# ZJU-FAST-Lab/Implicit-SDF-Planner

Hardware: AMD Instinct MI355X
Metric: SDF cost+grad point-evals/sec (higher is better)
Workload: dtype f64; 1 GPU; V3 ESDF-tile sweep: 1 trajectory x 40 pieces x 65 samples/piece, 256^3 fp32 ESDF @ 0.2 m, kernel_size 21, box robot (1.6,0.3,0.3) central-diff grad, occ_thresh = 0, cull off = BASELINE configs[1]; pieces=40, samples_per_piece=65, grid=256, kernel_size=21, collective=none

## Files before the change

### implicit-sdf-planner_amd/csrc/isdf_host.hip

```cpp
#include "isdf_ctx.hpp"
#include "minco_dev.hpp"
#include "lbfgs_host.hpp"
#include <array>
#include <atomic>
#include <map>
#include <dlfcn.h>
#include <chrono>
#include <cmath>
#include <cstdio>
#include <cstring>
#include <functional>
#include <cstdlib>
#include <string>
#include <vector>
#include <new>
#include "fwn_host.hpp"

using namespace isdf;

namespace {
thread_local std::string g_create_error;
}

int isdf_fail(isdf_ctx *c, int code, const char *msg) {
// ... 731 lines not shown
static int rebuild_bit_grids(isdf_ctx *c, const isdf_config &cfg, SweepParams &P, hipStream_t st) {
    const int zw = (c->grid.Z + 31) / 32, xw = (c->grid.X + 31) / 32, yw = (c->grid.Y + 31) / 32;
    const size_t nwz = (size_t)c->grid.X * c->grid.Y * zw, nwx = (size_t)c->grid.Y * c->grid.Z * xw, nwy = (size_t)c->grid.X * c->grid.Z * yw;
    { const int rc = c->d_bits.reserve(c, nwz + nwx + nwy); if (rc) return rc; }
    c->grid.ZW = zw; c->grid.XW = xw; c->grid.YW = yw;
    c->grid.bits = c->d_bits; c->grid.bits_x = c->d_bits + nwz; c->grid.bits_y = c->d_bits + nwz + nwx;
    launch_build_bits(c->grid, cfg.variant == ISDF_V3_ESDF_TILE ? 1 : 0, cfg.occ_thresh, c->d_bits, st);
    launch_build_bits_xy(c->grid, cfg.variant == ISDF_V3_ESDF_TILE ? 1 : 0, cfg.occ_thresh, c->d_bits + nwz, c->d_bits + nwz + nwx, st);
    c->bits_dirty = false;
    P.grid = c->grid;
    return ISDF_OK;
}

static int plan_order(isdf_ctx *c, const isdf_config &cfg, SweepParams &P, bool fused, long long pb, long long pe, long long total_pieces, hipStream_t st) {
    const int N = P.N;
    P.plan_cls_in = nullptr; P.plan_cls_out = nullptr; P.plan_map_out = nullptr; P.plan_zone = 0; P.plan_group = 1;
    P.plan_lr_in = P.plan_hist_in = nullptr; P.plan_lr_out = P.plan_hist_out = nullptr;
    const int K1 = cfg.integral_intervs + 1;
    const long long n_loc = pe - pb, ns_local = n_loc * K1;
    const int nb = (int)((ns_local + 3) / 4);
    P.n_sweep_blocks = nb;
    if (c->n_cus == 0) { hipDeviceProp_t pr; c->n_cus = (hipGetDeviceProperties(&pr, c->device) == hipSuccess && pr.multiProcessorCount > 0) ? pr.multiProcessorCount : 256; }
    const bool no_plan = c->env_no_lpt;
    bool plan = cfg.enable_pos && !no_plan && !P.sample_map && K1 <= 128 && nb > c->n_cus && ns_local < (1LL << 28) && c->shape.kind != ISDF_SHAPE_MESH;
    long long group = n_loc;
    int zone = 0;
    if (plan) {
        if (fused) {
            plan = P.xf.world <= 1 && pb == 0 && pe == total_pieces && ns_local <= PLAN_GROUP_MAX_SAMPLES;
            zone = c->n_cus;
        } else if (nb <= sweep_resident_blocks(P, c->n_cus) && ns_local <= PLAN_GROUP_MAX_SAMPLES) {
// ... 10 lines not shown
        c->plan_ns_cap = c->plan_np_cap = 0; c->plan_k = 0; c->plan_cur = 0;
        const size_t nsc = std::max(ns_cap, (size_t)4096), npc = std::max(np_cap, (size_t)256);
        HIPCHK(c, c->d_plan_cls.alloc(2 * nsc));
        HIPCHK(c, c->d_plan_map.alloc(2 * nsc));
        HIPCHK(c, c->d_plan_lr.alloc(2 * nsc));
        HIPCHK(c, c->d_plan_hist.alloc(2 * npc * PLAN_CLASSES));
        c->plan_ns_cap = nsc; c->plan_np_cap = npc;
    }
    const long long geo = ((long long)n_loc << 32) | ((long long)K1 << 20) | ((long long)(fused ? 1 : 0) << 19) | (long long)(group & 0x7FFFF);
    if (c->plan_ns != ns_local || c->plan_nb != nb || c->plan_geo != geo) { c->plan_k = 0; c->plan_ns = ns_local; c->plan_nb = nb; c->plan_geo = geo; }
    constexpr int PLAN_CYCLE = 8;
    const int k = c->plan_k, ph = k % PLAN_CYCLE;
    const size_t nsc = c->plan_ns_cap;
    P.plan_zone = zone;
    P.plan_group = (int)group;
    if (ph == 0) P.plan_cls_out = c->d_plan_cls;
    if (ph == 1) { P.plan_cls_in = c->d_plan_cls; P.plan_lr_out = c->d_plan_lr; P.plan_hist_out = c->d_plan_hist; }
    if (ph == 2) { P.plan_lr_in = c->d_plan_lr; P.plan_hist_in = c->d_plan_hist; P.plan_map_out = c->d_plan_map + (size_t)(1 - c->plan_cur) * nsc; }
    if (ph == 3) c->plan_cur = 1 - c->plan_cur;
    if (k >= 3) P.sample_map = c->d_plan_map + (size_t)c->plan_cur * nsc;
    if (c->plan_k < (1 << 30)) c->plan_k++;
    return ISDF_OK;
}

static int mesh_queue(isdf_ctx *c, const isdf_config &cfg, SweepParams &P, size_t ns_loc) {
    const double k3 = (double)cfg.kernel_size * cfg.kernel_size * cfg.kernel_size;
    double vox = k3;
    if (c->shape.prune_rows) {
        double v = 1.0;
        for (int a = 0; a < 3; a++) v *= ((double)c->shape.bbox_hi[a] - (double)c->shape.bbox_lo[a] + 2.2 * cfg.safety_hor) / P.grid.res + 3.0;
// ... 61 lines not shown
    P.bd_half = cfg.kernel_size * P.grid.res / 2;
    P.safety_hor = cfg.safety_hor; P.weight_p = cfg.weight_p; P.weight_v = cfg.weight_v; P.weight_omg = cfg.weight_omg;
    P.weight_theta = cfg.weight_theta;
    P.vel_sqr_max = cfg.vmax * cfg.vmax; P.omg_sqr_max = cfg.omgmax * cfg.omgmax; P.theta_max = cfg.thetamax;
    P.mu = cfg.smoothing_eps; P.inv_mu = 1.0 / cfg.smoothing_eps; P.inv_K = 1.0 / cfg.integral_intervs;
    P.occ_thresh = (float)cfg.occ_thresh;
    P.cull_threshold = 0.0;
    if (cfg.variant == ISDF_V3_ESDF_TILE && cfg.enable_cull && c->shape.bound_radius > 0)
        P.cull_threshold = c->shape.bound_radius + cfg.safety_hor + std::sqrt(3.0) * P.grid.res + (cfg.occ_thresh > 0 ? cfg.occ_thresh : 0.0);
    P.T = d_T; P.coeffs = d_coeffs; P.acc = c->d_acc; P.sample_info = c->d_sample_info; P.piece_cost = c->d_piece_cost;
    P.out = d_out; P.stats = c->d_stats;
    P.dbg = nullptr;
    P.sample_map = (c->d_sample_map && c->sample_map_n == 4 * ((ns_loc + 3) / 4)) ? c->d_sample_map.get() : nullptr;
    P.dbg_flags = 0;
    if (const char *e = getenv("ISDF_DEBUG_FLAGS")) P.dbg_flags = atoi(e);
    rc = debug_timing_buffer(c, n_samples * 8 + (size_t)total_pieces * 4 + 4, st, &P.dbg);
    if (rc) return rc;
    if (cfg.enable_pos && c->bits_dirty) { rc = rebuild_bit_grids(c, cfg, P, st); if (rc) return rc; }
    c->last_P = P; c->have_last_P = true;
    ProfEvent *ev;
    rc = prof_begin(c, st, &ev);
    if (rc) return rc;
    if (ev && !cfg.enable_pos) { ev = nullptr; c->prof_used--; }
    const bool ev2 = ev && c->prof_secondary;
    const bool fused = c->fuse_small && !ev2 && sweep_can_fuse(P);
    {
        int xerr = ISDF_OK;
        if (isdf_xchg_fill(c, &P.xf, (size_t)total_pieces, &xerr)) {
            if (xerr != ISDF_OK) return xerr;
        }
    }
// ... 1078 lines not shown
    (void)hipSetDevice(c->device);
    (void)hipDeviceSynchronize();
    c->d_sample_map.release(); c->sample_map_n = 0;
    if (!map || n <= 0) return ISDF_OK;
    if (c->d_sample_map.alloc((size_t)n) != hipSuccess) return ISDF_ERR_HIP;
    (void)hipMemcpy(c->d_sample_map, map, (size_t)n * sizeof(int), hipMemcpyHostToDevice);
    c->sample_map_n = (size_t)n;
    return ISDF_OK;
}

extern "C" int isdf_debug_plan_map(isdf_ctx *c, int *out, long long cap) {
    if (!c || c->plan_k < 4 || !c->d_plan_map) return 0;
    (void)hipSetDevice(c->device);
    (void)hipDeviceSynchronize();
    const long long n = 4LL * c->plan_nb < cap ? 4LL * c->plan_nb : cap;
    if (out && n > 0) (void)hipMemcpy(out, c->d_plan_map + (size_t)c->plan_cur * c->plan_ns_cap, (size_t)n * sizeof(int), hipMemcpyDeviceToHost);
    return c->plan_k;
}

extern "C" long long isdf_debug_sample_info(isdf_ctx *c, int *out, long long cap) {
    if (!c || !c->d_sample_info || !c->have_last_P) return 0;
    (void)hipSetDevice(c->device);
    (void)hipDeviceSynchronize();
    const long long n = (long long)(c->last_P.piece_end - c->last_P.piece_begin) * (c->last_P.K + 1);
    const long long m = 2 * n < cap ? 2 * n : cap;
    if (out && m > 0) (void)hipMemcpy(out, c->d_sample_info, (size_t)m * sizeof(int), hipMemcpyDeviceToHost);
    return n;
}

extern "C" const char *isdf_debug_peek_hip_error(void) { return hipGetErrorString(hipPeekAtLastError()); }
```

### implicit-sdf-planner_amd/csrc/isdf_internal.hpp

```cpp
#pragma once
#include <hip/hip_runtime.h>
#include <hip/hip_ext.h>
#include <cstdint>
#include "dev_shapes.hpp"

namespace isdf {

struct DevGrid {
    int X, Y, Z;
    double res;
    double bmin[3], bmax[3];
    const float *esdf;
    const uint8_t *occ;
    const unsigned *bits;
    int ZW;
    const unsigned *bits_x;
    const unsigned *bits_y;
    int XW, YW;
};
constexpr int PLAN_CLASSES = 8;
constexpr int PLAN_GROUP_MAX_SAMPLES = 65535;
constexpr int ACC_STRIDE = 8;
constexpr int PARTIAL_STRIDE = 20;
constexpr int SWEPT_MAX_COARSE = 1536;
// ... 36 lines not shown
    unsigned long long *stats;
    const double *host_T, *host_coeffs;
    double *stage;
    unsigned long long *stage_flags;
    unsigned long long seq;
    unsigned long long *host_flag;
    void *poses;
    const int *sample_map;
    unsigned char *plan_cls_out;
    const unsigned char *plan_cls_in;
    unsigned short *plan_lr_out, *plan_hist_out;
    const unsigned short *plan_lr_in, *plan_hist_in;
    int *plan_map_out;
    int plan_zone;
    int plan_group;
    int dbg_flags;
    unsigned long long *dbg;
    unsigned *mq_entries;
    int2 *mq_items;
    double *mq_res;
    int *mq_sample_items;
    int *mq_sample_n;
    unsigned *mq_count;
    unsigned mq_cap;
    int mq_kmax;
};

size_t sweep_pose_bytes();
bool sweep_can_fuse(const SweepParams &P);
int sweep_resident_blocks(const SweepParams &P, int n_cus);
// ... 47 lines not shown
```

### implicit-sdf-planner_amd/csrc/tile_sweep.hip

```cpp
#define ISDF_LEAN_MATH 1
#ifndef ISDF_SWEEP_STATS
#define ISDF_SWEEP_STATS 0
#endif
#include "isdf_internal.hpp"
#include "dev_mesh.hpp"

namespace isdf {

constexpr int SW_LIST_CAP = 1024;
constexpr int MQ_BLOCK = 16;
constexpr int SW_PASS = 8;
constexpr int SW_NEAR_CAP = 512;
constexpr float TS_FILTER_EPS = 2e-3f;

__device__ __forceinline__ void wave_lds_sync() {
    __builtin_amdgcn_fence(__ATOMIC_RELEASE, "wavefront");
    __builtin_amdgcn_wave_barrier();
    __builtin_amdgcn_fence(__ATOMIC_ACQUIRE, "wavefront");
}

__device__ __forceinline__ bool in_map(const DevGrid &G, double x, double y, double z) {
    if (x < G.bmin[0] || y < G.bmin[1] || z < G.bmin[2]) return false;
    if (x > G.bmax[0] || y > G.bmax[1] || z > G.bmax[2]) return false;
    return true;
// ... 229 lines not shown
    const int n3 = nb - Z, p1 = pos - q0, w = p1 / n3;
    return w * nb + Z + (p1 - w * n3);
}
__device__ __forceinline__ uint4 plan_add(uint4 a, uint4 b) {
    return make_uint4(a.x + b.x, a.y + b.y, a.z + b.z, a.w + b.w);
}
__device__ __forceinline__ uint4 plan_wave_sum(uint4 v) {
#pragma unroll
    for (int d = 1; d < 64; d <<= 1) v = plan_add(v, make_uint4(__shfl_xor(v.x, d), __shfl_xor(v.y, d), __shfl_xor(v.z, d), __shfl_xor(v.w, d)));
    return v;
}
__device__ __forceinline__ unsigned plan_count(uint4 v, int q) {
    const unsigned w = (q >> 1) == 0 ? v.x : (q >> 1) == 1 ? v.y : (q >> 1) == 2 ? v.z : v.w;
    return (w >> (16 * (q & 1))) & 0xFFFFu;
}
__device__ void plan_wave(const SweepParams &P, const int t, const int lane) {
    const int K1 = P.K + 1, n_pieces = P.piece_end - P.piece_begin;
    const int ns = n_pieces * K1, nb = P.n_sweep_blocks, Z = P.plan_zone;
    const int G = P.plan_group, gp0 = (t / G) * G, gn = min(G, n_pieces - gp0);
    const int s0 = t * K1 + lane, s1 = s0 + 64;
    const bool h0 = lane < K1, h1 = lane + 64 < K1;
    if (P.plan_cls_in) {
        const int c0 = h0 ? (int)(P.plan_cls_in[s0] & (PLAN_CLASSES - 1)) : -1, c1 = h1 ? (int)(P.plan_cls_in[s1] & (PLAN_CLASSES - 1)) : -1;
        int r0 = 0, r1 = 0, hist = 0;
        const unsigned long long lt = (1ull << lane) - 1ull;
#pragma unroll
        for (int q = 0; q < PLAN_CLASSES; q++) {
            const unsigned long long m0 = __ballot(c0 == q), m1 = __ballot(c1 == q);
            if (c0 == q) r0 = __popcll(m0 & lt);
            if (c1 == q) r1 = __popcll(m0) + __popcll(m1 & lt);
// ... 9 lines not shown
            const uint4 h = reinterpret_cast<const uint4 *>(P.plan_hist_in)[i];
            tot = plan_add(tot, h);
            if (i < t) bef = plan_add(bef, h);
        }
        tot = plan_wave_sum(tot); bef = plan_wave_sum(bef);
        int base = 0;
        if (lane < PLAN_CLASSES) {
            base = (int)plan_count(bef, lane);
#pragma unroll
            for (int q = 1; q < PLAN_CLASSES; q++) if (q > lane) base += (int)plan_count(tot, q);
        }
        const unsigned v0 = h0 ? P.plan_lr_in[s0] : 0u, v1 = h1 ? P.plan_lr_in[s1] : 0u;
        const int b0 = __shfl(base, (int)(v0 & 7u)), b1 = __shfl(base, (int)(v1 & 7u));
        const int p0 = gp0 * K1 + b0 + (int)(v0 >> 3), p1 = gp0 * K1 + b1 + (int)(v1 >> 3);
        if (Z > 0) {
            if (h0) P.plan_map_out[plan_rank(p0, Z, nb)] = s0;
            if (h1) P.plan_map_out[plan_rank(p1, Z, nb)] = s1;
            if (t == 0) for (int pos = ns + lane; pos < 4 * nb; pos += 64) P.plan_map_out[plan_rank(pos, Z, nb)] = -1;
        } else {
            if (h0) P.plan_map_out[(p0 & 3) * nb + (p0 >> 2)] = s0;
            if (h1) P.plan_map_out[(p1 & 3) * nb + (p1 >> 2)] = s1;
            if (t == 0) for (int pos = ns + lane; pos < 4 * nb; pos += 64) P.plan_map_out[(pos & 3) * nb + (pos >> 2)] = -1;
        }
    }
}

constexpr int POSE_THREADS = 64;
constexpr int POSE_REC = (int)(sizeof(SweepPose) / 8);
__global__ __launch_bounds__(POSE_THREADS) void pose_kernel(const SweepParams P) {
    __shared__ double s_rec[POSE_THREADS][POSE_REC + 1];
    const int K1 = P.K + 1;
    const long long s_begin = (long long)P.piece_begin * K1, s_end = (long long)P.piece_end * K1;
// ... 77 lines not shown
    const int v0 = sa_w == 2 ? w0[1] : w0[2], v1 = sa_w == 2 ? w1[1] : w1[2];
    sp.rx0 = (flags_w & 1) ? u0 : 0; sp.ry0 = (flags_w & 1) ? v0 : 0;
    sp.rnx = (flags_w & 1) ? max(0, u1 - u0 + 1) : 0; sp.rny = (flags_w & 1) ? max(0, v1 - v0 + 1) : 0;
    sp.nzt = sa_w == 2 ? nn[2] : (sa_w == 0 ? nn[0] : nn[1]);
    sp.flags = flags_w;
    sp.sa = sa_w;
    scan_consts(P, scan_launch_consts(P, P.shape.kind), sp.pos, sp.R, sp.lo, sa_w, sp.rny, P.shape.kind == ISDF_SHAPE_ROUNDEDCONE && P.shape.f.ident != 0, sp);
    }
    __syncthreads();
    const int n_rec = (int)min((long long)POSE_THREADS, s_end - s_first);
    double *dst = (double *)((SweepPose *)P.poses + (s_first - s_begin));
    for (int i = threadIdx.x; i < n_rec * POSE_REC; i += POSE_THREADS) dst[i] = s_rec[i / POSE_REC][i % POSE_REC];
}
size_t sweep_pose_bytes() { return sizeof(SweepPose); }

template <bool EARLY, bool XF> __device__ __forceinline__ void tail_piece(const SweepParams &P, const int t, double (*s_val)[PARTIAL_STRIDE + 1]);

template <int KIND, bool IDENT, bool FUSED>
__global__ __launch_bounds__(64 * SW_SAMPLES, FUSED ? 3 : sweep_waves_per_simd(KIND, IDENT)) void sweep_kernel(const SweepParams P) {
    const int n_blocks = FUSED ? P.n_sweep_blocks : (int)gridDim.x;
    if constexpr (FUSED) {
        __shared__ double s_tail[TL_THREADS][PARTIAL_STRIDE + 1];
        if ((int)blockIdx.x >= n_blocks) {
            if ((P.plan_cls_in || P.plan_lr_in) && !(P.dbg_flags & 2) && (threadIdx.x >> 6) == SW_SAMPLES - 1) plan_wave(P, (int)blockIdx.x - n_blocks, threadIdx.x & 63);
            if (P.xf.world > 1) tail_piece<false, true>(P, (int)blockIdx.x - n_blocks, s_tail);
            else tail_piece<false, false>(P, (int)blockIdx.x - n_blocks, s_tail);
            return;
        }
    }
    if constexpr (FUSED) {
        if (P.host_T && (int)blockIdx.x < (P.n_traj * P.N + STAGE_G - 1) / STAGE_G) stage_in(P, (int)blockIdx.x);
    }
    __shared__ SweepPose s_pose[SW_SAMPLES];
    __shared__ unsigned s_list[SW_SAMPLES][SW_LIST_CAP];
    __shared__ unsigned s_near[SW_SAMPLES][SW_NEAR_CAP];
    __shared__ __attribute__((aligned(16))) int s_plan[SW_SAMPLES][4];
    __shared__ double s_res[SW_SAMPLES][SW_NEAR_CAP / 64][ACC_STRIDE];
    __shared__ int s_resn[SW_SAMPLES][SW_NEAR_CAP / 64][2];
    __shared__ __attribute__((aligned(8))) unsigned s_mframes[KIND == ISDF_SHAPE_MESH ? SW_SAMPLES : 1][KIND == ISDF_SHAPE_MESH ? mesh_frames_words(MESH_Q_LEVELS) : 2];

    const int lane = threadIdx.x & 63;
    const int wave = __builtin_amdgcn_readfirstlane(threadIdx.x >> 6);
    const int K1 = P.K + 1;
    const long long s_begin = (long long)P.piece_begin * K1, s_end = (long long)P.piece_end * K1;
    const DevGrid &G = P.grid;
    const long long rank_w = (long long)blockIdx.x + (long long)wave * n_blocks;
    long long sidx = s_begin + rank_w;
    if (P.sample_map) { const int m = __builtin_amdgcn_readfirstlane(P.sample_map[rank_w]); sidx = m >= 0 ? s_begin + m : s_end; }
    unsigned long long *const dbg = (ISDF_SWEEP_STATS && P.dbg && sidx < s_end) ? P.dbg + (size_t)(sidx - s_begin) * 8 : nullptr;
    if (dbg && lane == 0) { dbg[0] = wall_clock64(); dbg[1] = clock64(); }

    auto sample_of_rank = [&](long long rank) -> long long {
        if (P.sample_map) { const int m = P.sample_map[rank]; return m >= 0 ? s_begin + m : s_end; }
        return s_begin + rank;
    };
    if constexpr (FUSED) {
    long long pose_sidx = s_end;
    if (wave == 0 && lane < SW_SAMPLES) pose_sidx = sample_of_rank((long long)blockIdx.x + (long long)lane * n_blocks);
    if (pose_sidx < s_end) {
        const SampleId id = decode_sample(P, pose_sidx);
        bool staged = true;
        if constexpr (FUSED) if (P.host_T) staged = stage_wait(P, id.b * P.N + id.i);
        if (!staged && P.stats) atomicMax(&P.stats[4], 1ull);
        const PieceIn pin = piece_in(P, id.b, id.i);
        const double *c = pin.c;
        const int ld = pin.ld;
        const double step = pin.T * P.inv_K;
        Basis B;
        poly_basis(id.j * step, B);
        const d3 pos = ct_beta(c, ld, B.b0), vel = ct_beta<1>(c, ld, B.b1), acc = ct_beta<2>(c, ld, B.b2);
        FlatS fs;
        flat_core(P.flat, vel, acc, fs);
        const d4 quat = flat_quat(fs);
        const m3 R = quat_to_rot(quat);
        SweepPose &sp = s_pose[lane];
        sp.pos[0] = pos.x; sp.pos[1] = pos.y; sp.pos[2] = pos.z;
#pragma unroll
        for (int k = 0; k < 9; k++) sp.R[k] = R.a[k];
        sp.quat[0] = quat.w; sp.quat[1] = quat.x; sp.quat[2] = quat.y; sp.quat[3] = quat.z;
        int flags = 0;
        if (P.enable_pos) {
            flags = 1;
// ... 6 lines not shown
            const double hb[3] = {0.5 * ((double)P.shape.bbox_hi[0] - (double)P.shape.bbox_lo[0]) + infl,
                                  0.5 * ((double)P.shape.bbox_hi[1] - (double)P.shape.bbox_lo[1]) + infl,
                                  0.5 * ((double)P.shape.bbox_hi[2] - (double)P.shape.bbox_lo[2]) + infl};
            const double cb[3] = {0.5 * ((double)P.shape.bbox_hi[0] + (double)P.shape.bbox_lo[0]),
                                  0.5 * ((double)P.shape.bbox_hi[1] + (double)P.shape.bbox_lo[1]),
                                  0.5 * ((double)P.shape.bbox_hi[2] + (double)P.shape.bbox_lo[2])};
            const double p[3] = {pos.x, pos.y, pos.z};
#pragma unroll
            for (int a = 0; a < 3; a++) {
                const double ctr = p[a] + R.a[3 * a] * cb[0] + R.a[3 * a + 1] * cb[1] + R.a[3 * a + 2] * cb[2];
                const double ext = fabs(R.a[3 * a]) * hb[0] + fabs(R.a[3 * a + 1]) * hb[1] + fabs(R.a[3 * a + 2]) * hb[2];
                sp.L0[a] = (ctr - ext - G.bmin[a]) * inv_res - 0.5;
                sp.L1[a] = (ctr + ext - G.bmin[a]) * inv_res - 0.5;
            }
        }
    }
    if (wave == 1 && lane < 3 * SW_SAMPLES && P.enable_pos) {
        const int ps = lane / 3, a = lane - 3 * ps;
        const long long sx = sample_of_rank((long long)blockIdx.x + (long long)ps * n_blocks);
        if (sx < s_end) {
            const SampleId id = decode_sample(P, sx);
            if constexpr (FUSED) if (P.host_T) (void)stage_wait(P, id.b * P.N + id.i);
            const PieceIn pin = piece_in(P, id.b, id.i);
            const double step = pin.T * P.inv_K;
            Basis B;
            poly_basis(id.j * step, B);
            const double *ca = pin.c + (size_t)a * pin.ld;
            double pa = 0.0;
#pragma unroll
            for (int k = 0; k < 6; k++) pa += ca[k] * B.b0[k];
            const double bmn = a == 0 ? G.bmin[0] : (a == 1 ? G.bmin[1] : G.bmin[2]), bmx = a == 0 ? G.bmax[0] : (a == 1 ? G.bmax[1] : G.bmax[2]);
            const int dim = a == 0 ? G.X : (a == 1 ? G.Y : G.Z);
            const int lo = axis_index(clampd(pa - P.bd_half, bmn, bmx), bmn, G.res, dim);
            const int hi = axis_index(clampd(pa + P.bd_half, bmn, bmx), bmn, G.res, dim);
            s_pose[ps].lo[a] = lo;
            s_pose[ps].nn[a] = hi - lo + 1;
// ... 118 lines not shown
        for (int a = 0; a < 3; a++) { Ru[a] = w.Ru[a]; Rv[a] = w.Rv[a]; Rw[a] = w.Rw[a]; dzv[a] = w.dzv[a]; dzi[a] = w.dzi[a]; }
        pv_u = w.pvu; pv_v = w.pvv; pv_w = w.pvw; inv_rny = w.inv_rny;
        cone_alpha = w.cone_alpha; cone_ia = w.cone_ia; cone_on = w.cone_on != 0;
    } else {
#pragma unroll
        for (int k = 0; k < 9; k++) Rf[k] = rec->Rf[k];
        pvx = rec->pv[0]; pvy = rec->pv[1]; pvz = rec->pv[2];
#pragma unroll
        for (int a = 0; a < 3; a++) { Ru[a] = rec->Ru[a]; Rv[a] = rec->Rv[a]; Rw[a] = rec->Rw[a]; dzv[a] = rec->dzv[a]; dzi[a] = rec->dzi[a]; }
        pv_u = rec->pvu; pv_v = rec->pvv; pv_w = rec->pvw; inv_rny = rec->inv_rny;
        cone_alpha = rec->cone_alpha; cone_ia = rec->cone_ia; cone_on = rec->cone_on != 0;
#pragma unroll
        for (int a = 0; a < 3; a++) { asm volatile("" : "+v"(dzv[a])); asm volatile("" : "+v"(dzi[a])); }
    }
    const float cone_A = SL.cone_A, cone_B = SL.cone_B;

    auto row_xy = [&](int t) -> unsigned {
        unsigned wx = (unsigned)((float)t * inv_rny);
        int rem = t - (int)wx * rny;
        if (rem < 0) { wx--; rem += rny; } else if (rem >= rny) { wx++; rem -= rny; }
        const unsigned wy = (unsigned)rem;
        return ((wx + (unsigned)rx0) << sh_u) | ((wy + (unsigned)ry0) << sh_v);
    };
    auto row_bits = [&](unsigned pk, int zb) -> unsigned {
        const int z0 = lo_w + (zb << 5);
        const int nz = min(32, nzt - (zb << 5));
        const size_t rowbase = ((size_t)(lo_u + (int)((pk >> sh_u) & 1023u)) * dim_v + (lo_v + (int)((pk >> sh_v) & 1023u))) * n_ww;
        const int w0 = z0 >> 5, sh = z0 & 31;
        const unsigned b0 = bits_a[rowbase + w0];
        const unsigned b1 = bits_a[rowbase + min(w0 + 1, n_ww - 1)];
// ... 478 lines not shown
    const int K1 = P.K + 1;
    const long long n_samples = (long long)(P.piece_end - P.piece_begin) * K1;
    unsigned long long culled = 0, pairs = 0, grads = 0;
    if (P.enable_pos)
        for (long long s = (long long)blockIdx.x * blockDim.x + threadIdx.x; s < n_samples; s += (long long)gridDim.x * blockDim.x) {
            const int a = P.sample_info[2 * s], b = P.sample_info[2 * s + 1];
            pairs += (unsigned)a; grads += (unsigned)(b & 0x7fffffff);
            if (b < 0) culled++;
        }
    if (culled) atomicAdd(&P.stats[1], culled);
    if (pairs) atomicAdd(&P.stats[2], pairs);
    if (grads) atomicAdd(&P.stats[3], grads);
    if (blockIdx.x == 0 && threadIdx.x == 0) atomicAdd(&P.stats[0], (unsigned long long)n_samples);
}

template <bool EARLY, bool XF> __device__ __forceinline__ void tail_piece(const SweepParams &P, const int t, double (*s_val)[PARTIAL_STRIDE + 1]) {
    const int K1 = P.K + 1;
    const int tid = threadIdx.x;
    const int n_own = P.piece_end - P.piece_begin;
    int gp = t;
    if constexpr (XF) gp = t < n_own ? P.piece_begin + t : (t - n_own < P.piece_begin ? t - n_own : t);
    const int b = gp / P.N, i = gp - b * P.N;
    const size_t ostride = (size_t)1 + 19 * (size_t)P.N;
    const int p0 = max(P.piece_begin, b * P.N) - b * P.N, p1 = min(P.piece_end, (b + 1) * P.N) - b * P.N;
    double *const o = P.out + (size_t)b * ostride;
    double *const my_board = XF ? P.xf.board[P.xf.rank] + (size_t)P.xf.parity * P.xf.parity_stride : nullptr;
    bool lost = false;
    const bool mine = i >= p0 && i < p1;
    unsigned long long *const dbg = (ISDF_SWEEP_STATS && P.dbg && mine) ? P.dbg + (size_t)(P.piece_end - P.piece_begin) * K1 * 8 + (size_t)(gp - P.piece_begin) * 4 : nullptr;
    if (!mine) {
        const int q = tid;
        if constexpr (XF) {
            if (q < 19) {
                double v;
                unsigned long long deadline = 0ull;
                lost = !xslot_take(my_board + (size_t)gp * XF_ROW + q, v, P.xf.timeout_ticks, deadline);
                if (q == 18) o[1 + i] = v;
                else { const int d = q / 6, r = q - 6 * d; o[1 + P.N + (size_t)d * 6 * P.N + 6 * i + r] = v; }
            }
        } else {
            if (q == 18) o[1 + i] = 0.0;
            else if (q < 18) { const int d = q / 6, r = q - 6 * d; o[1 + P.N + (size_t)d * 6 * P.N + 6 * i + r] = 0.0; }
            else if (q == 19 && p1 <= p0 && i == 0) o[0] = 0.0;
            return;
// ... 1 lines not shown
    } else {
    if constexpr (!EARLY) {
        if (P.host_T) {
            __shared__ int s_staged;
            if (tid == 0) s_staged = stage_wait(P, gp) ? 1 : 0;
            __syncthreads();
            lost = lost || !s_staged;
        }
    }
    const PieceIn pin = piece_in(P, b, i);
    const double *c = pin.c;
    const int ld = pin.ld;
    const double integral_frac = P.inv_K;
    const double step = pin.T * integral_frac;
    double colsum = 0.0;
    unsigned long long tl_c0 = 0, tl_marks = 0;
    if (dbg && tid == 0) { dbg[0] = wall_clock64(); tl_c0 = clock64(); }
#define TL_MARK(k) do { if (dbg && tid == 0) tl_marks |= (((clock64() - tl_c0) >> 4) & 0xFFFFull) << (16 * (k)); } while (0)
    for (int j0 = 0; j0 < (EARLY ? K1 : min(K1, 1)); j0 += TL_THREADS) {
        const int j = j0 + tid;
        if (tid < TL_THREADS && j < K1) {
            const long long s = (long long)gp * K1 + j;
            double *const ap = P.acc + (size_t)(s - (long long)P.piece_begin * K1) * ACC_STRIDE;
            double ab[EARLY ? ACC_STRIDE : 1];
            if (EARLY && P.enable_pos) {
#pragma unroll
                for (int q = 0; q < ACC_STRIDE; q++) ab[q] = ap[q];
            }
            d3 vel, acc3, jer0;
            {
                Basis B;
                poly_basis(j * step, B);
                vel = ct_beta<1>(c, ld, B.b1); acc3 = ct_beta<2>(c, ld, B.b2); jer0 = ct_beta<3>(c, ld, B.b3);
            }
            TL_MARK(0);
            double pena = 0.0;
            d3 gradVel = mk3(0, 0, 0), gradPos = gradVel, gradOmg = gradVel;
            d4 gradQuat; gradQuat.w = gradQuat.x = gradQuat.y = gradQuat.z = 0.0;
            FlatS fs; FlatS2 ft;
            flat_core(P.flat, vel, acc3, fs);
            flat_core2(P.flat, vel, acc3, jer0, fs, ft);
            if (P.enable_dyn) {
                const d4 quat = flat_quat(fs);
                const d3 omg = flat_omg(fs, ft);
                const double cos_theta = 1.0 - 2.0 * (quat.x * quat.x + quat.y * quat.y);
                const double violaVel = dot3(vel, vel) - P.vel_sqr_max;
                const double violaOmg = dot3(omg, omg) - P.omg_sqr_max;
                const double violaTheta = acos(cos_theta) - P.theta_max;
// ... 35 lines not shown
                }
                if (a[0] > 0.0) {
                    gradPos.x += P.weight_p * a[1]; gradPos.y += P.weight_p * a[2]; gradPos.z += P.weight_p * a[3];
                    gradQuat.w += P.weight_p * a[4]; gradQuat.x += P.weight_p * a[5];
                    gradQuat.y += P.weight_p * a[6]; gradQuat.z += P.weight_p * a[7];
                    pena += P.weight_p * a[0];
                }
            }
            d3 gP, gV, gA, gJ;
            TL_MARK(2);
            flat_backward_from(P.flat, vel, acc3, fs, ft, gradPos, gradVel, gradQuat, gradOmg, gP, gV, gA, gJ);
            TL_MARK(3);
            const double node = (j == 0 || j == P.K) ? 0.5 : 1.0;
            const double alpha = j * integral_frac;
            double *o = s_val[tid];
            double s1 = j * step;
            asm volatile("" : "+v"(s1));
            Basis B;
            poly_basis(s1, B);
            const d3 jer = ct_beta<3>(c, ld, B.b3), sna = ct_beta<4>(c, ld, B.b4);
            const double gPv[3] = {gP.x, gP.y, gP.z}, gVv[3] = {gV.x, gV.y, gV.z}, gAv[3] = {gA.x, gA.y, gA.z}, gJv[3] = {gJ.x, gJ.y, gJ.z};
#pragma unroll
            for (int d = 0; d < 3; d++)
#pragma unroll
                for (int r = 0; r < 6; r++) {
                    double v = B.b0[r] * gPv[d];
                    if (r >= 1) v += B.b1[r] * gVv[d];
                    if (r >= 2) v += B.b2[r] * gAv[d];
                    if (r >= 3) v += B.b3[r] * gJv[d];
                    o[d * 6 + r] = v * node * step;
                }
            o[18] = (dot3(gP, vel) + dot3(gV, acc3) + dot3(gA, jer) + dot3(gJ, sna)) * alpha * node * step + node * integral_frac * pena;
            o[19] = node * step * pena;
        }
        __syncthreads();
        {
            const int n = min(TL_THREADS, K1 - j0);
            const int col = tid % PARTIAL_STRIDE, grp = tid / PARTIAL_STRIDE;
            double part = 0.0;
            if (grp < TL_GROUPS) for (int row = grp; row < n; row += TL_GROUPS) part += s_val[row][col];
            __syncthreads();
            if (grp < TL_GROUPS) s_val[grp][col] = part;
            __syncthreads();
            if (tid < PARTIAL_STRIDE) {
#pragma unroll
                for (int g = 0; g < TL_GROUPS; g++) colsum += s_val[g][tid];
            }
        }
        __syncthreads();
    }
    if (dbg && tid == 0) { dbg[2] = tl_marks; dbg[3] = (clock64() - tl_c0) >> 4; }
#undef TL_MARK
    if (P.host_flag) lost = __syncthreads_or(lost ? 1 : 0) != 0;
    if (tid < PARTIAL_STRIDE) {
        const int q = tid;
        if (q < 19) {
            if (q == 18) o[1 + i] = colsum;
            else { const int d = q / 6, r = q - 6 * d; o[1 + P.N + (size_t)d * 6 * P.N + 6 * i + r] = colsum; }
            if constexpr (XF) {
                for (int r = 0; r < P.xf.world; r++)
                    if (r != P.xf.rank) xslot_publish(P.xf.board[r] + (size_t)P.xf.parity * P.xf.parity_stride + (size_t)gp * XF_ROW + q, colsum);
            }
        } else {
            if (P.host_flag) { if (lost && P.stats) atomicMax(&P.stats[4], 1ull); __builtin_amdgcn_fence(__ATOMIC_RELEASE, ""); }
            if constexpr (XF) {
                for (int r = 0; r < P.xf.world; r++) xslot_publish(P.xf.board[r] + (size_t)P.xf.parity * P.xf.parity_stride + (size_t)gp * XF_ROW + 19, colsum);
            } else slot_publish(&P.piece_cost[gp], colsum);
        }
    }
    }
    if (lost && P.stats) atomicMax(&P.stats[4], 1ull);
    bool collector;
    int k0, k1;
    if constexpr (XF) {
        const int first = b * P.N, last = first + P.N - 1;
        const int t_last = (last >= P.piece_begin && last < P.piece_end) ? last - P.piece_begin : (last < P.piece_begin ? last + n_own : last);
        const int below = P.piece_begin - 1;
        const int t_below = (below >= first && below <= last) ? below + n_own : -1;
        collector = t == max(t_last, t_below);
        k0 = 0; k1 = P.N;
    } else {
        collector = i == p1 - 1;
        k0 = p0; k1 = p1;
    }
// ... 16 lines not shown
                v = __longlong_as_double((long long)bits);
            }
            sum += v;
        }
        sum = wave_sum(sum);
        if (__ballot(gone) != 0ull) { sum = __longlong_as_double(0x7FF8000000000000ll); if (tid == 0 && P.stats) atomicMax(&P.stats[4], 1ull); }
        if (tid == 0) o[0] = sum;
    }
    if constexpr (!XF) {
        if (P.host_flag && collector && tid == 0) {
            __builtin_amdgcn_fence(__ATOMIC_ACQUIRE, "agent");
            const unsigned long long ovf = P.stats ? __hip_atomic_load(&P.stats[4], __ATOMIC_RELAXED, __HIP_MEMORY_SCOPE_AGENT) : 0ull;
            __hip_atomic_store(&P.host_flag[b], P.seq | (ovf ? HOST_FLAG_OVERFLOW : 0ull), __ATOMIC_RELEASE, __HIP_MEMORY_SCOPE_SYSTEM);
        }
    }
    if (dbg && tid == 0) dbg[1] = wall_clock64();
}

constexpr int TL_LAUNCH_THREADS = TL_THREADS + 64;
template <bool XF> __device__ __forceinline__ void tail_plan(const SweepParams &P) {
    if (!(P.plan_cls_in || P.plan_lr_in) || (P.dbg_flags & 2) || (int)(threadIdx.x >> 6) != TL_THREADS / 64) return;
    int gp = (int)blockIdx.x;
    if constexpr (XF) { const int n_own = P.piece_end - P.piece_begin, t = gp; gp = t < n_own ? P.piece_begin + t : (t - n_own < P.piece_begin ? t - n_own : t); }
    if (gp >= P.piece_begin && gp < P.piece_end) plan_wave(P, gp - P.piece_begin, (int)(threadIdx.x & 63));
}
__global__ __launch_bounds__(TL_LAUNCH_THREADS) void tail_kernel(const SweepParams P) {
    __shared__ double s_val[TL_THREADS][PARTIAL_STRIDE + 1];
    tail_plan<false>(P);
    tail_piece<true, false>(P, (int)blockIdx.x, s_val);
}
__global__ __launch_bounds__(TL_LAUNCH_THREADS) void tail_kernel_xf(const SweepParams P) {
    __shared__ double s_val[TL_THREADS][PARTIAL_STRIDE + 1];
    tail_plan<true>(P);
    tail_piece<true, true>(P, (int)blockIdx.x, s_val);
}

static int fused_max_blocks() {
    static const int v = [] { const char *e = getenv("ISDF_FUSE_MAX_BLOCKS"); const int n = e ? atoi(e) : 0; return n > 0 ? n : 3 * 256; }();
    return v;
}

int sweep_resident_blocks(const SweepParams &P, int n_cus) {
    const bool ident = P.shape.d.ident != 0;
    const int kind = P.shape.kind == ISDF_SHAPE_MESH ? ISDF_SHAPE_MESH : P.shape.kind;
    return sweep_waves_per_simd(kind, kind == ISDF_SHAPE_MESH ? false : ident) * n_cus;
}

bool sweep_can_fuse(const SweepParams &P) {
    if (!P.enable_pos || P.shape.kind == ISDF_SHAPE_MESH || P.shape.d.ident == 0) return false;
// ... 105 lines not shown
```

Baseline: 162.4 million point-evals/s.

## Pack plan map entries, park tail basis values in LDS, overlay fused tail reduction

In fused mode, each plan-map entry is now packed as (piece<<7)|sample, so the sweep can get piece and sample indices with shifts and no integer division. The fused tail stores the polynomial basis terms and the jerk/snap vectors in its shared-memory row during the first pass, so the second pass reuses them instead of recomputing the basis. Its reduction writes partial sums into the otherwise unused s_res buffer, which the sweep's large shared arrays now share, and this removes two __syncthreads barriers. It also adds debug timing marks, which are compiled only when stats are enabled.

```diff
diff --git a/implicit-sdf-planner_amd/csrc/isdf_host.hip b/implicit-sdf-planner_amd/csrc/isdf_host.hip
--- a/implicit-sdf-planner_amd/csrc/isdf_host.hip
+++ b/implicit-sdf-planner_amd/csrc/isdf_host.hip
@@ -769,7 +769,7 @@
 
 static int plan_order(isdf_ctx *c, const isdf_config &cfg, SweepParams &P, bool fused, long long pb, long long pe, long long total_pieces, hipStream_t st) {
     const int N = P.N;
-    P.plan_cls_in = nullptr; P.plan_cls_out = nullptr; P.plan_map_out = nullptr; P.plan_zone = 0; P.plan_group = 1;
+    P.plan_cls_in = nullptr; P.plan_cls_out = nullptr; P.plan_map_out = nullptr; P.plan_zone = 0; P.plan_group = 1; P.plan_packed = 0;
     P.plan_lr_in = P.plan_hist_in = nullptr; P.plan_lr_out = P.plan_hist_out = nullptr;
     const int K1 = cfg.integral_intervs + 1;
     const long long n_loc = pe - pb, ns_local = n_loc * K1;
@@ -810,6 +810,7 @@
     const size_t nsc = c->plan_ns_cap;
     P.plan_zone = zone;
     P.plan_group = (int)group;
+    P.plan_packed = (fused && n_loc < (1LL << 23)) ? 1 : 0;
     if (ph == 0) P.plan_cls_out = c->d_plan_cls;
     if (ph == 1) { P.plan_cls_in = c->d_plan_cls; P.plan_lr_out = c->d_plan_lr; P.plan_hist_out = c->d_plan_hist; }
     if (ph == 2) { P.plan_lr_in = c->d_plan_lr; P.plan_hist_in = c->d_plan_hist; P.plan_map_out = c->d_plan_map + (size_t)(1 - c->plan_cur) * nsc; }
@@ -901,7 +902,7 @@
     P.sample_map = (c->d_sample_map && c->sample_map_n == 4 * ((ns_loc + 3) / 4)) ? c->d_sample_map.get() : nullptr;
     P.dbg_flags = 0;
     if (const char *e = getenv("ISDF_DEBUG_FLAGS")) P.dbg_flags = atoi(e);
-    rc = debug_timing_buffer(c, n_samples * 8 + (size_t)total_pieces * 4 + 4, st, &P.dbg);
+    rc = debug_timing_buffer(c, n_samples * 12 + (size_t)total_pieces * 8 + 4, st, &P.dbg);
     if (rc) return rc;
     if (cfg.enable_pos && c->bits_dirty) { rc = rebuild_bit_grids(c, cfg, P, st); if (rc) return rc; }
     c->last_P = P; c->have_last_P = true;
@@ -2010,7 +2011,12 @@
     (void)hipSetDevice(c->device);
     (void)hipDeviceSynchronize();
     const long long n = 4LL * c->plan_nb < cap ? 4LL * c->plan_nb : cap;
-    if (out && n > 0) (void)hipMemcpy(out, c->d_plan_map + (size_t)c->plan_cur * c->plan_ns_cap, (size_t)n * sizeof(int), hipMemcpyDeviceToHost);
+    if (out && n > 0) {
+        (void)hipMemcpy(out, c->d_plan_map + (size_t)c->plan_cur * c->plan_ns_cap, (size_t)n * sizeof(int), hipMemcpyDeviceToHost);
+        const int K1 = (int)((c->plan_geo >> 20) & 0xFFF);
+        if ((c->plan_geo >> 19) & 1)
+            for (long long i = 0; i < n; i++) if (out[i] >= 0) out[i] = (out[i] >> 7) * K1 + (out[i] & 127);
+    }
     return c->plan_k;
 }
 
diff --git a/implicit-sdf-planner_amd/csrc/isdf_internal.hpp b/implicit-sdf-planner_amd/csrc/isdf_internal.hpp
--- a/implicit-sdf-planner_amd/csrc/isdf_internal.hpp
+++ b/implicit-sdf-planner_amd/csrc/isdf_internal.hpp
@@ -74,6 +74,7 @@
     int *plan_map_out;
     int plan_zone;
     int plan_group;
+    int plan_packed;
     int dbg_flags;
     unsigned long long *dbg;
     unsigned *mq_entries;
diff --git a/implicit-sdf-planner_amd/csrc/tile_sweep.hip b/implicit-sdf-planner_amd/csrc/tile_sweep.hip
--- a/implicit-sdf-planner_amd/csrc/tile_sweep.hip
+++ b/implicit-sdf-planner_amd/csrc/tile_sweep.hip
@@ -267,6 +267,7 @@
     const unsigned w = (q >> 1) == 0 ? v.x : (q >> 1) == 1 ? v.y : (q >> 1) == 2 ? v.z : v.w;
     return (w >> (16 * (q & 1))) & 0xFFFFu;
 }
+__device__ __forceinline__ int plan_entry_sample(const SweepParams &P, int m, int K1) { return P.plan_packed ? (m >> 7) * K1 + (m & 127) : m; }
 __device__ void plan_wave(const SweepParams &P, const int t, const int lane) {
     const int K1 = P.K + 1, n_pieces = P.piece_end - P.piece_begin;
     const int ns = n_pieces * K1, nb = P.n_sweep_blocks, Z = P.plan_zone;
@@ -306,8 +307,8 @@
         const int b0 = __shfl(base, (int)(v0 & 7u)), b1 = __shfl(base, (int)(v1 & 7u));
         const int p0 = gp0 * K1 + b0 + (int)(v0 >> 3), p1 = gp0 * K1 + b1 + (int)(v1 >> 3);
         if (Z > 0) {
-            if (h0) P.plan_map_out[plan_rank(p0, Z, nb)] = s0;
-            if (h1) P.plan_map_out[plan_rank(p1, Z, nb)] = s1;
+            if (h0) P.plan_map_out[plan_rank(p0, Z, nb)] = P.plan_packed ? ((t << 7) | lane) : s0;
+            if (h1) P.plan_map_out[plan_rank(p1, Z, nb)] = P.plan_packed ? ((t << 7) | (lane + 64)) : s1;
             if (t == 0) for (int pos = ns + lane; pos < 4 * nb; pos += 64) P.plan_map_out[plan_rank(pos, Z, nb)] = -1;
         } else {
             if (h0) P.plan_map_out[(p0 & 3) * nb + (p0 >> 2)] = s0;
@@ -415,17 +416,23 @@
 }
 size_t sweep_pose_bytes() { return sizeof(SweepPose); }
 
-template <bool EARLY, bool XF> __device__ __forceinline__ void tail_piece(const SweepParams &P, const int t, double (*s_val)[PARTIAL_STRIDE + 1]);
+template <bool EARLY, bool XF> __device__ __forceinline__ void tail_piece(const SweepParams &P, const int t, double (*s_val)[PARTIAL_STRIDE + 1], double *s_part);
+constexpr int TL_PARK = 20;
+static_assert(TL_PARK <= PARTIAL_STRIDE, "a thread parks in its own row");
 
 template <int KIND, bool IDENT, bool FUSED>
 __global__ __launch_bounds__(64 * SW_SAMPLES, FUSED ? 3 : sweep_waves_per_simd(KIND, IDENT)) void sweep_kernel(const SweepParams P) {
     const int n_blocks = FUSED ? P.n_sweep_blocks : (int)gridDim.x;
+    __shared__ unsigned s_list[SW_SAMPLES][SW_LIST_CAP];
+    __shared__ unsigned s_near[SW_SAMPLES][SW_NEAR_CAP];
+    __shared__ double s_res[SW_SAMPLES][SW_NEAR_CAP / 64][ACC_STRIDE];
     if constexpr (FUSED) {
         __shared__ double s_tail[TL_THREADS][PARTIAL_STRIDE + 1];
         if ((int)blockIdx.x >= n_blocks) {
             if ((P.plan_cls_in || P.plan_lr_in) && !(P.dbg_flags & 2) && (threadIdx.x >> 6) == SW_SAMPLES - 1) plan_wave(P, (int)blockIdx.x - n_blocks, threadIdx.x & 63);
-            if (P.xf.world > 1) tail_piece<false, true>(P, (int)blockIdx.x - n_blocks, s_tail);
-            else tail_piece<false, false>(P, (int)blockIdx.x - n_blocks, s_tail);
+            static_assert(sizeof(s_res) >= TL_GROUPS * (PARTIAL_STRIDE + 1) * 8, "overlay of the fused tail");
+            if (P.xf.world > 1) tail_piece<false, true>(P, (int)blockIdx.x - n_blocks, s_tail, &s_res[0][0][0]);
+            else tail_piece<false, false>(P, (int)blockIdx.x - n_blocks, s_tail, &s_res[0][0][0]);
             return;
         }
     }
@@ -433,10 +440,7 @@
         if (P.host_T && (int)blockIdx.x < (P.n_traj * P.N + STAGE_G - 1) / STAGE_G) stage_in(P, (int)blockIdx.x);
     }
     __shared__ SweepPose s_pose[SW_SAMPLES];
-    __shared__ unsigned s_list[SW_SAMPLES][SW_LIST_CAP];
-    __shared__ unsigned s_near[SW_SAMPLES][SW_NEAR_CAP];
     __shared__ __attribute__((aligned(16))) int s_plan[SW_SAMPLES][4];
-    __shared__ double s_res[SW_SAMPLES][SW_NEAR_CAP / 64][ACC_STRIDE];
     __shared__ int s_resn[SW_SAMPLES][SW_NEAR_CAP / 64][2];
     __shared__ __attribute__((aligned(8))) unsigned s_mframes[KIND == ISDF_SHAPE_MESH ? SW_SAMPLES : 1][KIND == ISDF_SHAPE_MESH ? mesh_frames_words(MESH_Q_LEVELS) : 2];
 
@@ -447,19 +451,34 @@
     const DevGrid &G = P.grid;
     const long long rank_w = (long long)blockIdx.x + (long long)wave * n_blocks;
     long long sidx = s_begin + rank_w;
-    if (P.sample_map) { const int m = __builtin_amdgcn_readfirstlane(P.sample_map[rank_w]); sidx = m >= 0 ? s_begin + m : s_end; }
+    if (P.sample_map) { const int m = __builtin_amdgcn_readfirstlane(P.sample_map[rank_w]); sidx = m >= 0 ? s_begin + plan_entry_sample(P, m, K1) : s_end; }
     unsigned long long *const dbg = (ISDF_SWEEP_STATS && P.dbg && sidx < s_end) ? P.dbg + (size_t)(sidx - s_begin) * 8 : nullptr;
     if (dbg && lane == 0) { dbg[0] = wall_clock64(); dbg[1] = clock64(); }
-
-    auto sample_of_rank = [&](long long rank) -> long long {
-        if (P.sample_map) { const int m = P.sample_map[rank]; return m >= 0 ? s_begin + m : s_end; }
-        return s_begin + rank;
+    [[maybe_unused]] const auto dbg_ext = [&](long long s) -> unsigned long long * {
+        return P.dbg + (size_t)(s_end - s_begin) * 8 + (size_t)(P.piece_end - P.piece_begin) * 4 + 4 + (size_t)(s - s_begin) * 4;
+    };
+
+    [[maybe_unused]] auto sample_of_rank = [&](long long rank) -> SampleId {
+        if (P.sample_map && P.plan_packed) {
+            const int m = P.sample_map[rank];
+            SampleId id;
+            const int gp = P.piece_begin + (m >> 7);
+            id.j = m & 127;
+            id.b = P.n_traj == 1 ? 0 : gp / P.N;
+            id.i = gp - id.b * P.N;
+            id.s = m >= 0 ? (long long)gp * K1 + id.j : s_end;
+            return id;
+        }
+        long long s = s_begin + rank;
+        if (P.sample_map) { const int m = P.sample_map[rank]; s = m >= 0 ? s_begin + m : s_end; }
+        return decode_sample(P, s);
     };
     if constexpr (FUSED) {
-    long long pose_sidx = s_end;
-    if (wave == 0 && lane < SW_SAMPLES) pose_sidx = sample_of_rank((long long)blockIdx.x + (long long)lane * n_blocks);
+    SampleId id;
+    id.s = s_end; id.b = id.i = id.j = 0;
+    if (wave == 0 && lane < SW_SAMPLES) id = sample_of_rank((long long)blockIdx.x + (long long)lane * n_blocks);
+    const long long pose_sidx = id.s;
     if (pose_sidx < s_end) {
-        const SampleId id = decode_sample(P, pose_sidx);
         bool staged = true;
         if constexpr (FUSED) if (P.host_T) staged = stage_wait(P, id.b * P.N + id.i);
         if (!staged && P.stats) atomicMax(&P.stats[4], 1ull);
@@ -467,6 +486,14 @@
         const double *c = pin.c;
         const int ld = pin.ld;
         const double step = pin.T * P.inv_K;
+#if ISDF_SWEEP_STATS
+        if (P.dbg) {
+            double all = step;
+            for (int d = 0; d < 3; d++) for (int k = 0; k < 6; k++) all += c[(size_t)d * ld + k];
+            asm volatile("" :: "v"(all));
+            dbg_ext(pose_sidx)[0] = clock64();
+        }
+#endif
         Basis B;
         poly_basis(id.j * step, B);
         const d3 pos = ct_beta(c, ld, B.b0), vel = ct_beta<1>(c, ld, B.b1), acc = ct_beta<2>(c, ld, B.b2);
@@ -503,12 +530,14 @@
                 sp.L1[a] = (ctr + ext - G.bmin[a]) * inv_res - 0.5;
             }
         }
+#if ISDF_SWEEP_STATS
+        if (P.dbg) { asm volatile("s_waitcnt lgkmcnt(0)" ::: "memory"); dbg_ext(pose_sidx)[1] = clock64(); }
+#endif
     }
     if (wave == 1 && lane < 3 * SW_SAMPLES && P.enable_pos) {
         const int ps = lane / 3, a = lane - 3 * ps;
-        const long long sx = sample_of_rank((long long)blockIdx.x + (long long)ps * n_blocks);
-        if (sx < s_end) {
-            const SampleId id = decode_sample(P, sx);
+        const SampleId id = sample_of_rank((long long)blockIdx.x + (long long)ps * n_blocks);
+        if (id.s < s_end) {
             if constexpr (FUSED) if (P.host_T) (void)stage_wait(P, id.b * P.N + id.i);
             const PieceIn pin = piece_in(P, id.b, id.i);
             const double step = pin.T * P.inv_K;
@@ -657,6 +686,9 @@
         for (int a = 0; a < 3; a++) { asm volatile("" : "+v"(dzv[a])); asm volatile("" : "+v"(dzi[a])); }
     }
     const float cone_A = SL.cone_A, cone_B = SL.cone_B;
+#if ISDF_SWEEP_STATS
+    if (dbg && lane == 0 && !primed) { float all = pvx + pvy + pvz + pv_u + pv_v + pv_w + inv_rny + dzi[0] + dzi[1] + dzi[2] + cone_ia; asm volatile("" :: "v"(all)); dbg_ext(sidx)[2] = clock64(); }
+#endif
 
     auto row_xy = [&](int t) -> unsigned {
         unsigned wx = (unsigned)((float)t * inv_rny);
@@ -1165,7 +1197,7 @@
     if (blockIdx.x == 0 && threadIdx.x == 0) atomicAdd(&P.stats[0], (unsigned long long)n_samples);
 }
 
-template <bool EARLY, bool XF> __device__ __forceinline__ void tail_piece(const SweepParams &P, const int t, double (*s_val)[PARTIAL_STRIDE + 1]) {
+template <bool EARLY, bool XF> __device__ __forceinline__ void tail_piece(const SweepParams &P, const int t, double (*s_val)[PARTIAL_STRIDE + 1], double *s_part) {
     const int K1 = P.K + 1;
     const int tid = threadIdx.x;
     const int n_own = P.piece_end - P.piece_begin;
@@ -1179,6 +1211,8 @@
     bool lost = false;
     const bool mine = i >= p0 && i < p1;
     unsigned long long *const dbg = (ISDF_SWEEP_STATS && P.dbg && mine) ? P.dbg + (size_t)(P.piece_end - P.piece_begin) * K1 * 8 + (size_t)(gp - P.piece_begin) * 4 : nullptr;
+    [[maybe_unused]] unsigned long long *const dbg2 = dbg ? P.dbg + (size_t)n_own * K1 * 12 + (size_t)n_own * 4 + 4 + (size_t)(gp - P.piece_begin) * 4 : nullptr;
+    [[maybe_unused]] unsigned long long tl_c0 = 0, tl_marks2 = 0;
     if (!mine) {
         const int q = tid;
         if constexpr (XF) {
@@ -1210,9 +1244,10 @@
     const double integral_frac = P.inv_K;
     const double step = pin.T * integral_frac;
     double colsum = 0.0;
-    unsigned long long tl_c0 = 0, tl_marks = 0;
+    unsigned long long tl_marks = 0;
     if (dbg && tid == 0) { dbg[0] = wall_clock64(); tl_c0 = clock64(); }
 #define TL_MARK(k) do { if (dbg && tid == 0) tl_marks |= (((clock64() - tl_c0) >> 4) & 0xFFFFull) << (16 * (k)); } while (0)
+#define TL_MARK2(k) do { if (ISDF_SWEEP_STATS && dbg && tid == 0) tl_marks2 |= (((clock64() - tl_c0) >> 4) & 0xFFFFull) << (16 * (k)); } while (0)
     for (int j0 = 0; j0 < (EARLY ? K1 : min(K1, 1)); j0 += TL_THREADS) {
         const int j = j0 + tid;
         if (tid < TL_THREADS && j < K1) {
@@ -1228,6 +1263,13 @@
                 Basis B;
                 poly_basis(j * step, B);
                 vel = ct_beta<1>(c, ld, B.b1); acc3 = ct_beta<2>(c, ld, B.b2); jer0 = ct_beta<3>(c, ld, B.b3);
+                if constexpr (!EARLY) {
+                    const d3 sna0 = ct_beta<4>(c, ld, B.b4);
+                    const double pk[TL_PARK] = {B.b0[1], B.b0[2], B.b0[3], B.b0[4], B.b0[5], B.b1[2], B.b1[3], B.b1[4], B.b1[5], B.b2[3], B.b2[4], B.b2[5],
+                                                B.b3[4], B.b3[5], jer0.x, jer0.y, jer0.z, sna0.x, sna0.y, sna0.z};
+#pragma unroll
+                    for (int k = 0; k < TL_PARK; k++) s_val[tid][k] = pk[k];
+                }
             }
             TL_MARK(0);
             double pena = 0.0;
@@ -1293,11 +1335,24 @@
             const double node = (j == 0 || j == P.K) ? 0.5 : 1.0;
             const double alpha = j * integral_frac;
             double *o = s_val[tid];
-            double s1 = j * step;
-            asm volatile("" : "+v"(s1));
             Basis B;
-            poly_basis(s1, B);
-            const d3 jer = ct_beta<3>(c, ld, B.b3), sna = ct_beta<4>(c, ld, B.b4);
+            d3 jer, sna;
+            if constexpr (EARLY) {
+                double s1 = j * step;
+                asm volatile("" : "+v"(s1));
+                poly_basis(s1, B);
+                jer = ct_beta<3>(c, ld, B.b3); sna = ct_beta<4>(c, ld, B.b4);
+            } else {
+                double pk[TL_PARK];
+#pragma unroll
+                for (int k = 0; k < TL_PARK; k++) pk[k] = o[k];
+                poly_basis(0.0, B);
+                B.b0[1] = pk[0]; B.b0[2] = pk[1]; B.b0[3] = pk[2]; B.b0[4] = pk[3]; B.b0[5] = pk[4];
+                B.b1[2] = pk[5]; B.b1[3] = pk[6]; B.b1[4] = pk[7]; B.b1[5] = pk[8];
+                B.b2[3] = pk[9]; B.b2[4] = pk[10]; B.b2[5] = pk[11];
+                B.b3[4] = pk[12]; B.b3[5] = pk[13];
+                jer = mk3(pk[14], pk[15], pk[16]); sna = mk3(pk[17], pk[18], pk[19]);
+            }
             const double gPv[3] = {gP.x, gP.y, gP.z}, gVv[3] = {gV.x, gV.y, gV.z}, gAv[3] = {gA.x, gA.y, gA.z}, gJv[3] = {gJ.x, gJ.y, gJ.z};
 #pragma unroll
             for (int d = 0; d < 3; d++)
@@ -1311,6 +1366,7 @@
                 }
             o[18] = (dot3(gP, vel) + dot3(gV, acc3) + dot3(gA, jer) + dot3(gJ, sna)) * alpha * node * step + node * integral_frac * pena;
             o[19] = node * step * pena;
+            TL_MARK2(0);
         }
         __syncthreads();
         {
@@ -1318,18 +1374,19 @@
             const int col = tid % PARTIAL_STRIDE, grp = tid / PARTIAL_STRIDE;
             double part = 0.0;
             if (grp < TL_GROUPS) for (int row = grp; row < n; row += TL_GROUPS) part += s_val[row][col];
-            __syncthreads();
-            if (grp < TL_GROUPS) s_val[grp][col] = part;
+            double (*const s_sum)[PARTIAL_STRIDE + 1] = EARLY ? s_val : reinterpret_cast<double (*)[PARTIAL_STRIDE + 1]>(s_part);
+            if constexpr (EARLY) __syncthreads();
+            if (grp < TL_GROUPS) s_sum[grp][col] = part;
             __syncthreads();
             if (tid < PARTIAL_STRIDE) {
 #pragma unroll
-                for (int g = 0; g < TL_GROUPS; g++) colsum += s_val[g][tid];
-            }
-        }
-        __syncthreads();
+                for (int g = 0; g < TL_GROUPS; g++) colsum += s_sum[g][tid];
+            }
+        }
+        if constexpr (EARLY) __syncthreads();
     }
     if (dbg && tid == 0) { dbg[2] = tl_marks; dbg[3] = (clock64() - tl_c0) >> 4; }
-#undef TL_MARK
+    TL_MARK2(1);
     if (P.host_flag) lost = __syncthreads_or(lost ? 1 : 0) != 0;
     if (tid < PARTIAL_STRIDE) {
         const int q = tid;
@@ -1347,6 +1404,7 @@
             } else slot_publish(&P.piece_cost[gp], colsum);
         }
     }
+    TL_MARK2(2);
     }
     if (lost && P.stats) atomicMax(&P.stats[4], 1ull);
     bool collector;
@@ -1393,6 +1451,11 @@
             __hip_atomic_store(&P.host_flag[b], P.seq | (ovf ? HOST_FLAG_OVERFLOW : 0ull), __ATOMIC_RELEASE, __HIP_MEMORY_SCOPE_SYSTEM);
         }
     }
+#if ISDF_SWEEP_STATS
+    if (dbg && tid == 0) { TL_MARK2(3); dbg2[0] = tl_marks2; dbg2[1] = collector ? 1ull : 0ull; }
+#endif
+#undef TL_MARK
+#undef TL_MARK2
     if (dbg && tid == 0) dbg[1] = wall_clock64();
 }
 
@@ -1406,12 +1469,12 @@
 __global__ __launch_bounds__(TL_LAUNCH_THREADS) void tail_kernel(const SweepParams P) {
     __shared__ double s_val[TL_THREADS][PARTIAL_STRIDE + 1];
     tail_plan<false>(P);
-    tail_piece<true, false>(P, (int)blockIdx.x, s_val);
+    tail_piece<true, false>(P, (int)blockIdx.x, s_val, nullptr);
 }
 __global__ __launch_bounds__(TL_LAUNCH_THREADS) void tail_kernel_xf(const SweepParams P) {
     __shared__ double s_val[TL_THREADS][PARTIAL_STRIDE + 1];
     tail_plan<true>(P);
-    tail_piece<true, true>(P, (int)blockIdx.x, s_val);
+    tail_piece<true, true>(P, (int)blockIdx.x, s_val, nullptr);
 }
 
 static int fused_max_blocks() {
```

After: 164.0 million point-evals/s (median of 6 runs). 1.0% higher.
